# apache/incubator-predictionio

Measured on AMD Instinct MI355X. Metric: als_ratings_per_sec, higher is better.
Workload: dtype fp32; 1 GPU; model=als_rank64_implicit, global_batch=250000000, users=12500000, items=10000000, parallelism=dp1

## Files before the change

### predictionio_amd/ops/als.py

```python

from __future__ import annotations

from typing import Optional, Tuple

import torch

SUPPORTED_RANKS = (16, 32, 64, 128)


def pad_rank(f: int) -> int:
    for s in SUPPORTED_RANKS:
        if f <= s:
            return s
    raise ValueError(f"rank {f} > 128 not supported")


def gramian(Y: torch.Tensor) -> torch.Tensor:
    return Y.t() @ Y


def woodbury_lv(Y: torch.Tensor, YtY: torch.Tensor,
                lam: float) -> tuple:
    f = Y.shape[1]
    eye = torch.eye(f, dtype=Y.dtype, device=Y.device)
    B = YtY + lam * eye
    L = torch.linalg.cholesky(B)
    Linv = torch.linalg.solve_triangular(L, eye, upper=False)
    V = (Y @ Linv.mT).contiguous()
    import os as _os
    if (_os.environ.get("PIO_ALS_STAGE_BF16") == "1" and Y.is_cuda):
        V = V.to(torch.bfloat16).contiguous()
    return Linv, V


def als_solve(indptr: torch.Tensor, indices: torch.Tensor,
              values: torch.Tensor, Y: torch.Tensor,
              YtY: Optional[torch.Tensor] = None,
              lam: float = 0.01, alpha: float = 1.0,
              implicit: bool = False, wr_scale: bool = True,
              lv: Optional[tuple] = None,
              row_range: Optional[Tuple[int, int]] = None,
              out: Optional[torch.Tensor] = None) -> torch.Tensor:
    if implicit:
        wr_scale = False
        if YtY is None:
            YtY = gramian(Y)
    if row_range is not None:
        lo, hi = row_range
        indptr = indptr[lo:hi + 1]
    if Y.is_cuda:
        from predictionio_amd.ops import hip_ext
        ext = hip_ext()
        f = Y.shape[1]
        pf = pad_rank(f)
        Yp = (Y if pf == f
              else torch.nn.functional.pad(Y, (0, pf - f))).contiguous()
        YtYp = None
        if YtY is not None:
            YtYp = (YtY if pf == f
                    else torch.nn.functional.pad(YtY, (0, pf - f, 0, pf - f))
                    ).contiguous()
        ip, ix, vv = (indptr.contiguous(), indices.contiguous(),
                      values.contiguous())
        if ix.numel():
            mx = int(ix.max())
            if mx >= Y.shape[0] or int(ix.min()) < 0:
                raise ValueError(
                    f"CSR column id out of range: [{int(ix.min())}, {mx}]"
                    f" vs {Y.shape[0]} factor rows")
        direct_out = (out if out is not None and pf == f
                      and out.is_contiguous() else None)
        if implicit and pf <= 128:
            if lv is not None:
                Linv, V = lv
            else:
                Linv, V = woodbury_lv(Yp, YtYp, lam)
            import os as _os
            if _os.environ.get("PIO_ALS_STAGE_BF16") == "1" \
                    and V.dtype == torch.float32:
                V = V.to(torch.bfloat16).contiguous()
            Z = ext.als_solve(ip, ix, vv, Yp, YtYp, V, float(lam),
                              float(alpha), True, False, 1, None)
            if direct_out is not None:
                X = direct_out
                torch.matmul(Z, Linv, out=X)
            else:
                X = (Z @ Linv).contiguous()
            ext.als_solve(ip, ix, vv, Yp, YtYp, None, float(lam),
                          float(alpha), True, False, 2, X)
        else:
            X = ext.als_solve(ip, ix, vv, Yp, YtYp, None, float(lam),
                              float(alpha), bool(implicit), bool(wr_scale),
                              0, direct_out)
        res = X[:, :f].contiguous() if pf != f else X
        if out is not None and res.data_ptr() != out.data_ptr():
            out.copy_(res)
            return out
        return res
    res = als_solve_ref(indptr, indices, values, Y, YtY, lam, alpha,
                        implicit, wr_scale)
    if out is not None:
        out.copy_(res)
        return out
    return res


def prepare_lv(Y: torch.Tensor, YtY: torch.Tensor, lam: float):
    f = Y.shape[1]
    pf = pad_rank(f)
    Yp = (Y if pf == f
          else torch.nn.functional.pad(Y, (0, pf - f))).contiguous()
    YtYp = (YtY if pf == f
            else torch.nn.functional.pad(YtY, (0, pf - f, 0, pf - f))
            ).contiguous()
    return woodbury_lv(Yp, YtYp, lam)


def als_solve_ref(indptr, indices, values, Y, YtY=None, lam=0.01, alpha=1.0,
                  implicit=False, wr_scale=True) -> torch.Tensor:
    n_rows = indptr.shape[0] - 1
    f = Y.shape[1]
    X = torch.zeros((n_rows, f), dtype=Y.dtype, device=Y.device)
    eye = torch.eye(f, dtype=Y.dtype, device=Y.device)
    ip = indptr.tolist()
    for r in range(n_rows):
        s, e = ip[r], ip[r + 1]
        nnz = e - s
        if implicit:
            A = (YtY if YtY is not None else gramian(Y)).clone()
            b = torch.zeros(f, dtype=Y.dtype, device=Y.device)
            if nnz:
                cols = indices[s:e].long()
                Yr = Y[cols]
                v = values[s:e]
                A = A + (Yr.t() * (alpha * v)) @ Yr
                b = Yr.t() @ (1.0 + alpha * v)
            A = A + lam * eye
        else:
            if nnz == 0:
                continue
            cols = indices[s:e].long()
            Yr = Y[cols]
            v = values[s:e]
            A = Yr.t() @ Yr + lam * (nnz if wr_scale else 1.0) * eye
            b = Yr.t() @ v
        X[r] = torch.linalg.solve(A, b)
    return X


def build_csr(rows: torch.Tensor, cols: torch.Tensor, vals: torch.Tensor,
              n_rows: int) -> Tuple[torch.Tensor, torch.Tensor, torch.Tensor]:
    order = torch.argsort(rows)
    r = rows[order]
    indices = cols[order].to(torch.int32)
    values = vals[order].to(torch.float32)
    counts = torch.bincount(r.long(), minlength=n_rows)
    indptr = torch.zeros(n_rows + 1, dtype=torch.int64, device=rows.device)
    torch.cumsum(counts, 0, out=indptr[1:])
    return indptr, indices, values


def aggregate_ratings(rows: torch.Tensor, cols: torch.Tensor,
                      vals: torch.Tensor, n_cols: int,
                      mode: str = "sum"):
    key = rows.long() * n_cols + cols.long()
    if mode == "sum":
        uk, inv = torch.unique(key, return_inverse=True)
        out = torch.zeros(uk.numel(), dtype=torch.float32, device=vals.device)
        out.scatter_add_(0, inv, vals.float())
    elif mode == "latest":
        sk, order = torch.sort(key, stable=True)
        last = torch.ones(sk.numel(), dtype=torch.bool, device=key.device)
        last[:-1] = sk[1:] != sk[:-1]
        uk = sk[last]
        out = vals[order][last].float()
    else:
        raise ValueError(mode)
    return (uk // n_cols).to(rows.dtype), (uk % n_cols).to(cols.dtype), out
```

### predictionio_amd/ops/build.py

```python

from __future__ import annotations

import os
import subprocess
import sys
import sysconfig

OPS_DIR = os.path.dirname(os.path.abspath(__file__))
CSRC = os.path.join(OPS_DIR, "csrc")
SO_PATH = os.path.join(OPS_DIR, "_pio_hip.so")
SOURCES = ["bindings.cpp", "als_kernels.hip", "topk_kernels.hip",
           "topk_mfma.hip"]
HEADERS = ["topk_common.h"]
ARCH = os.environ.get("PYTORCH_ROCM_ARCH", "gfx950")


def _torch_paths():
    import torch
    root = os.path.dirname(torch.__file__)
    return {
        "includes": [
            os.path.join(root, "include"),
            os.path.join(root, "include", "torch", "csrc", "api", "include"),
        ],
        "libdir": os.path.join(root, "lib"),
        "abi": int(torch._C._GLIBCXX_USE_CXX11_ABI),
    }


def needs_build() -> bool:
    if not os.path.exists(SO_PATH):
        return True
    so_mtime = os.path.getmtime(SO_PATH)
    for s in SOURCES + HEADERS:
        if os.path.getmtime(os.path.join(CSRC, s)) > so_mtime:
            return True
    return False


def build(force: bool = False, verbose: bool = True) -> str:
    if not force and not needs_build():
        return SO_PATH
    tp = _torch_paths()
    py_include = sysconfig.get_paths()["include"]
    hipcc = os.environ.get("HIPCC", "hipcc")
    cmd = [
        hipcc, f"--offload-arch={ARCH}", "-O3", "-std=c++17", "-fPIC",
        "-shared",
        "-DTORCH_EXTENSION_NAME=_pio_hip",
        "-DTORCH_API_INCLUDE_EXTENSION_H",
        f"-D_GLIBCXX_USE_CXX11_ABI={tp['abi']}",
        "-D__HIP_PLATFORM_AMD__=1", "-DUSE_ROCM=1",
        "-Wno-deprecated-declarations", "-Wno-unused-result",
        f"-I{py_include}",
    ]
    for inc in tp["includes"]:
        cmd.append(f"-I{inc}")
    cmd += [os.path.join(CSRC, s) for s in SOURCES]
    cmd += [
        f"-L{tp['libdir']}", f"-Wl,-rpath,{tp['libdir']}",
        "-ltorch", "-ltorch_cpu", "-ltorch_python", "-ltorch_hip",
        "-lc10", "-lc10_hip", "-lamdhip64",
        "-o", SO_PATH,
    ]
    if verbose:
        print("[ops.build]", " ".join(cmd), file=sys.stderr)
    subprocess.run(cmd, check=True)
    return SO_PATH


if __name__ == "__main__":
    build(force="--force" in sys.argv)
```

### predictionio_amd/ops/csrc/als_kernels.hip

```cpp

#include <hip/hip_runtime.h>

#define CHUNK 16

__device__ __forceinline__ void wave_sync() {
  __builtin_amdgcn_wave_barrier();
}

typedef __attribute__((ext_vector_type(4))) float f32x4_t;
typedef __attribute__((ext_vector_type(2))) float f32x2_t;

__device__ __forceinline__ f32x2_t fma2(f32x2_t a, f32x2_t b, f32x2_t c) {
  return __builtin_elementwise_fma(a, b, c);
}

__device__ __forceinline__ int uniform_i32(int v) {
  return __builtin_amdgcn_readfirstlane(v);
}
__device__ __forceinline__ long long uniform_i64(long long v) {
  const unsigned int lo = (unsigned int)uniform_i32((int)(unsigned long long)v);
  const unsigned int hi =
      (unsigned int)uniform_i32((int)((unsigned long long)v >> 32));
  return (long long)(((unsigned long long)hi << 32) | lo);
}
__device__ __forceinline__ float lane_bcast(float v, int k) {
  return __int_as_float(__builtin_amdgcn_readlane(__float_as_int(v), k));
}


template <int F>
__global__ __launch_bounds__(256) void als_solve_kernel(
    const long long* __restrict__ indptr,
    const int* __restrict__ indices,
    const float* __restrict__ values,
    const float* __restrict__ Y,
    const float* __restrict__ YtY,
    float* __restrict__ X,
    int n_rows,
    float lambda,
    float alpha,
    int implicit_mode,
    int wr_scale,
    int skip_below)
{
  constexpr int TM = 4;
  constexpr int TILES = (F / TM) * (F / TM);
  constexpr int TPT = (TILES + 255) / 256;
  constexpr int NB = 16;
  static_assert(F % TM == 0, "F must be divisible by 4");
  static_assert(F % NB == 0, "F must be divisible by the panel width");

  __shared__ float ys[CHUNK][F + 1];
  __shared__ float ws_a[CHUNK];
  __shared__ float ws_b[CHUNK];
  __shared__ float As[F][F + 4];
  __shared__ float bs[F];
  __shared__ float dinv_all[F];

  const int tid = threadIdx.x;
  const int lane = tid & 63;
  const int wave = tid >> 6;

  for (long long row = blockIdx.x; row < n_rows; row += gridDim.x) {
    const long long start = indptr[row];
    const long long end = indptr[row + 1];
    const int nnz = (int)(end - start);
    if (nnz <= skip_below) continue;

    float acc[TPT][TM][TM];
#pragma unroll
    for (int t = 0; t < TPT; ++t)
#pragma unroll
      for (int i = 0; i < TM; ++i)
#pragma unroll
        for (int j = 0; j < TM; ++j) acc[t][i][j] = 0.f;

    for (int i = tid; i < F; i += 256) bs[i] = 0.f;

    for (int base = 0; base < nnz; base += CHUNK) {
      const int cn = min(CHUNK, nnz - base);
      __syncthreads();
      for (int e = tid; e < cn * F; e += 256) {
        const int c = e / F;
        const int k = e % F;
        const int col = indices[start + base + c];
        ys[c][k] = Y[(long long)col * F + k];
      }
      if (tid < cn) {
        const float r = values[start + base + tid];
        if (implicit_mode) {
          ws_a[tid] = alpha * r;
          ws_b[tid] = 1.f + alpha * r;
        } else {
          ws_a[tid] = 1.f;
          ws_b[tid] = r;
        }
      }
      __syncthreads();

      if (tid < F) {
        float bacc = 0.f;
        for (int c = 0; c < cn; ++c) bacc += ws_b[c] * ys[c][tid];
        bs[tid] += bacc;
      }

#pragma unroll
      for (int t = 0; t < TPT; ++t) {
        const int tile = tid + t * 256;
        if (TILES >= 256 || tile < TILES) {
          const int ti = (tile / (F / TM)) * TM;
          const int tj = (tile % (F / TM)) * TM;
          for (int c = 0; c < cn; ++c) {
            const float w = ws_a[c];
            float ya[TM], yb[TM];
#pragma unroll
            for (int i = 0; i < TM; ++i) ya[i] = ys[c][ti + i];
#pragma unroll
            for (int j = 0; j < TM; ++j) yb[j] = ys[c][tj + j];
#pragma unroll
            for (int i = 0; i < TM; ++i)
#pragma unroll
              for (int j = 0; j < TM; ++j)
                acc[t][i][j] = fmaf(w * ya[i], yb[j], acc[t][i][j]);
          }
        }
      }
    }
    __syncthreads();

#pragma unroll
    for (int t = 0; t < TPT; ++t) {
      const int tile = tid + t * 256;
      if (TILES >= 256 || tile < TILES) {
        const int ti = (tile / (F / TM)) * TM;
        const int tj = (tile % (F / TM)) * TM;
#pragma unroll
        for (int i = 0; i < TM; ++i)
#pragma unroll
          for (int j = 0; j < TM; ++j) {
            float v = acc[t][i][j];
            if (YtY != nullptr) v += YtY[(ti + i) * F + (tj + j)];
            As[ti + i][tj + j] = v;
          }
      }
    }
    __syncthreads();
    if (tid < F) {
      const float reg = wr_scale ? lambda * (float)nnz : lambda;
      As[tid][tid] += reg;
    }
    __syncthreads();

    for (int k0 = 0; k0 < F; k0 += NB) {
      if (wave == 0) {
        for (int kk = 0; kk < NB; ++kk) {
          const int kq = k0 + kk;
          wave_sync();
          float d = As[kq][kq];
          d = d > 0.f ? sqrtf(d) : 1e-20f;
          const float dinv = 1.f / d;
          if (lane == kk) {
            As[kq][kq] = d;
            dinv_all[kq] = dinv;
// ... 230 lines not shown
          for (int r = 0; r < 4; ++r)
            Lc[wave][ti * 16 + lg * 4 + r][tj * 16 + lq] =
                accm[ti][tj][r];
      wave_sync();
#pragma unroll
      for (int m = 0; m < F; ++m) ap[m >> 1][m & 1] = Lc[wave][m][lane];
      wave_sync();
    } else {
    float yn[PD], vn[PD];
#pragma unroll
    for (int p = 0; p < PD; ++p) {
      if (p < nnz) {
        const int col = indices[start + p];
        yn[p] = lane < F ? Y[(long long)col * F + lane] : 0.f;
        vn[p] = values[start + p];
      }
    }
    for (int c0 = 0; c0 < nnz; c0 += PD) {
#pragma unroll
      for (int p = 0; p < PD; ++p) {
        const int c = c0 + p;
        if (c >= nnz) break;
        const float ycur = yn[p];
        const float vcur = vn[p];
        if (lane < F) ys[wave][p][lane] = ycur;
        wave_sync();
        if (c + PD < nnz) {
          const int ncol = indices[start + c + PD];
          if (lane < F) yn[p] = Y[(long long)ncol * F + lane];
          vn[p] = values[start + c + PD];
        }
        float w_a, w_b;
        if (implicit_mode) {
          w_a = alpha * vcur;
          w_b = 1.f + alpha * vcur;
        } else {
          w_a = 1.f;
          w_b = vcur;
        }
        b_reg = fmaf(w_b, ycur, b_reg);
        const float wyj = w_a * ycur;
        const f32x2_t wyj2 = {wyj, wyj};
#pragma unroll
        for (int q = 0; q < F / 4; ++q) {
          const f32x4_t y4 =
              *reinterpret_cast<const f32x4_t*>(&ys[wave][p][4 * q]);
          ap[2 * q + 0] = fma2(wyj2, y4.lo, ap[2 * q + 0]);
          ap[2 * q + 1] = fma2(wyj2, y4.hi, ap[2 * q + 1]);
        }
        wave_sync();
      }
    }

    }

    if (YtY != nullptr && lane < F) {
#pragma unroll
      for (int q = 0; q < F / 4; ++q) {
        const f32x4_t t4 = *reinterpret_cast<const f32x4_t*>(
            &YtY[(long long)lane * F + 4 * q]);
        ap[2 * q + 0] += t4.lo;
        ap[2 * q + 1] += t4.hi;
      }
    }
    {
      const float reg = wr_scale ? lambda * (float)nnz : lambda;
#pragma unroll
      for (int m = 0; m < F; ++m)
        if (m == ln) ap[m >> 1][m & 1] += reg;
    }

    float dl = 0.f;
#pragma unroll
    for (int k = 0; k < F; ++k) {
      float lkk = lane_bcast(ap[k >> 1][k & 1], k);
      lkk = lkk > 1e-30f ? lkk : 1e-30f;
      const float dinv = rsqrtf(lkk);
      const float ljk = ln > k ? ap[k >> 1][k & 1] * dinv : 0.f;
      dl = ln == k ? dinv : dl;
      Lc[wave][k][lane < F ? lane : F] = ljk;
      ap[k >> 1][k & 1] = ljk;
      wave_sync();
      const f32x2_t nl2 = {-ljk, -ljk};
#pragma unroll
      for (int m4 = (k + 1) & ~3; m4 < F; m4 += 4) {
        const f32x4_t lq =
            *reinterpret_cast<const f32x4_t*>(&Lc[wave][k][m4]);
        const f32x2_t lh[2] = {lq.lo, lq.hi};
#pragma unroll
        for (int h = 0; h < 2; ++h) {
          const int m2 = m4 + 2 * h;
          if (m2 > k)
            ap[m2 >> 1] = fma2(nl2, lh[h], ap[m2 >> 1]);
          else if (m2 == k)
            ap[m2 >> 1][1] = fmaf(-ljk, lh[h][1], ap[m2 >> 1][1]);
        }
      }
      wave_sync();
    }

#pragma unroll
    for (int k = 0; k < F; ++k) {
      const float zk = lane_bcast(b_reg * dl, k);
      b_reg = fmaf(-ap[k >> 1][k & 1], zk, b_reg);
    }
    b_reg *= dl;
    {
      float4 lq = {0.f, 0.f, 0.f, 0.f};
#pragma unroll
      for (int k = F - 1; k >= 0; --k) {
        if ((k & 3) == 3 && lane < F)
          lq = *reinterpret_cast<const float4*>(&Lc[wave][lane][k & ~3]);
        const float xk = lane_bcast(b_reg * dl, k);
        const float lv = (k & 3) == 0 ? lq.x
                         : (k & 3) == 1 ? lq.y
                         : (k & 3) == 2 ? lq.z : lq.w;
        b_reg = fmaf(ln < k ? -lv : 0.f, xk, b_reg);
      }
      b_reg *= dl;
    }

    if (lane < F) X[row * (long long)F + lane] = b_reg;
  }
}


#define WOODBURY_MAX_NNZ 32


template <int F, int NW, int NLO, bool BF16S = false>
__global__ __launch_bounds__(128, NW > 24 ? 5 : 6) void als_woodbury_kernel(
    const long long* __restrict__ indptr,
    const int* __restrict__ indices,
    const float* __restrict__ values,
    const float* __restrict__ Y,
    const float* __restrict__ V,
    float* __restrict__ X,
    int n_rows,
    float lambda,
    float alpha,
    int implicit_mode,
    int wr_scale,
    unsigned long long* prof)
{
  constexpr int FP = F + 4;
  constexpr int FPH = F + 8;
  const int lane = threadIdx.x & 63;
  const int wave = uniform_i32((int)(threadIdx.x >> 6));

  __shared__ float Yl[2][NW][BF16S ? (FPH / 2) : FP];
  constexpr int MP = NW + 4;
  __shared__ float M[2][NW][MP];
  __shared__ float tv[2][NW];
  __shared__ float dv[2][NW];

  float* yl = &Yl[wave][0][0];
  unsigned short* ylh = reinterpret_cast<unsigned short*>(yl);
  const float* src = implicit_mode ? V : Y;
  const unsigned short* srch = reinterpret_cast<const unsigned short*>(V);

  for (long long row = (long long)blockIdx.x * 2 + wave; row < n_rows;
       row += (long long)gridDim.x * 2) {
    const long long start = uniform_i64(indptr[row]);
    const int n = uniform_i32((int)(indptr[row + 1] - start));
    if (n > NW || n <= NLO) continue;
    if (n == 0 && NLO < 0) {
      for (int e = lane; e < F; e += 64)
        X[row * (long long)F + e] = 0.f;
      continue;
    }
    const bool probe = prof != nullptr && (row & 1023) == 0 && lane == 0;
    unsigned long long pt0 = 0, pt1 = 0, pt2 = 0, pt3 = 0;
    if (probe) pt0 = wall_clock64();

    if (lane < n)
      tv[wave][lane] = __int_as_float(indices[start + lane]);
    wave_sync();
    for (int c = 0; c < n; ++c) {
      const long long col = __float_as_int(tv[wave][c]);
      if constexpr (BF16S) {
        const unsigned int* srow = reinterpret_cast<const unsigned int*>(
            srch + col * F);
        unsigned int* drow =
            reinterpret_cast<unsigned int*>(ylh + c * FPH);
        for (int e = lane; e < F / 2; e += 64) drow[e] = srow[e];
      } else {
        for (int e = lane; e < F; e += 64)
          yl[c * FP + e] = src[col * F + e];
      }
    }
    if (lane < n) {
      const float r = values[start + lane];
      if (implicit_mode) {
        const float ar = alpha * r;
        const float d = sqrtf(ar > 1e-12f ? ar : 1e-12f);
        dv[wave][lane] = d;
        tv[wave][lane] = (1.f + ar) / d;
      } else {
        tv[wave][lane] = r;
      }
    }
    wave_sync();
    if (probe) pt1 = wall_clock64();

    const float reg = wr_scale ? lambda * (float)n : lambda;
    const int npairs = n * (n + 1) / 2;
    {
      int p = lane, i = 0;
      while (p >= n - i && i < n) { p -= n - i; ++i; }
      int j = i + p;
      for (int pp = lane; pp < npairs; pp += 64) {
        float dot;
        if constexpr (BF16S) {
          const uint4* yi8 = reinterpret_cast<const uint4*>(&ylh[i * FPH]);
          const uint4* yj8 = reinterpret_cast<const uint4*>(&ylh[j * FPH]);
          f32x4_t acc4 = {0.f, 0.f, 0.f, 0.f};
#pragma unroll
          for (int q = 0; q < F / 8; ++q) {
            const uint4 a = yi8[q];
            const uint4 b = yj8[q];
            const unsigned int av[4] = {a.x, a.y, a.z, a.w};
            const unsigned int bv[4] = {b.x, b.y, b.z, b.w};
#pragma unroll
            for (int t = 0; t < 4; ++t) {
              acc4.x = fmaf(__uint_as_float(av[t] << 16),
                            __uint_as_float(bv[t] << 16), acc4.x);
              acc4.y = fmaf(__uint_as_float(av[t] & 0xffff0000u),
                            __uint_as_float(bv[t] & 0xffff0000u), acc4.y);
            }
          }
          dot = acc4.x + acc4.y;
        } else {
          const f32x4_t* yi = reinterpret_cast<const f32x4_t*>(&yl[i * FP]);
          const f32x4_t* yj = reinterpret_cast<const f32x4_t*>(&yl[j * FP]);
          f32x4_t acc4 = {0.f, 0.f, 0.f, 0.f};
#pragma unroll
          for (int q = 0; q < F / 4; ++q) acc4 += yi[q] * yj[q];
          dot = acc4.x + acc4.y + acc4.z + acc4.w;
        }
        if (implicit_mode) {
          dot *= dv[wave][i] * dv[wave][j];
          if (i == j) dot += 1.f;
        } else if (i == j) {
          dot += reg;
        }
        M[wave][i][j] = dot;
        M[wave][j][i] = dot;
        j += 64;
        while (j >= n && i < n) { ++i; j -= n - i; }
      }
    }
    wave_sync();

    if (probe) pt2 = wall_clock64();
    const int ln = lane | (int)(start >> 63);
    f32x2_t mp[NW / 2];
    const float* mrow = &M[wave][lane < NW ? lane : NW - 1][0];
    const int wcol = lane < NW ? lane : NW;
#pragma unroll
    for (int q = 0; q < NW / 4; ++q) {
      const f32x4_t r4 = *reinterpret_cast<const f32x4_t*>(&mrow[4 * q]);
      mp[2 * q + 0] = lane < n ? r4.lo : f32x2_t{0.f, 0.f};
      mp[2 * q + 1] = lane < n ? r4.hi : f32x2_t{0.f, 0.f};
    }
    float t = lane < n ? tv[wave][lane] : 0.f;
    float dl = 0.f;
    wave_sync();
#pragma unroll
    for (int k = 0; k < NW; ++k) {
      if (k < n) {
        float mkk = lane_bcast(mp[k >> 1][k & 1], k);
        mkk = mkk > 1e-30f ? mkk : 1e-30f;
        const float dinv = rsqrtf(mkk);
        const float ljk = ln > k ? mp[k >> 1][k & 1] * dinv : 0.f;
        dl = ln == k ? dinv : dl;
        mp[k >> 1][k & 1] = ljk;
        M[wave][k][wcol] = ljk;
        wave_sync();
        const f32x2_t nl2 = {-ljk, -ljk};
#pragma unroll
        for (int j4 = (k + 1) & ~3; j4 < NW; j4 += 4) {
          const f32x4_t q4 =
              *reinterpret_cast<const f32x4_t*>(&M[wave][k][j4]);
          const f32x2_t qh[2] = {q4.lo, q4.hi};
#pragma unroll
          for (int h = 0; h < 2; ++h) {
            const int j2 = j4 + 2 * h;
            if (j2 > k)
              mp[j2 >> 1] = fma2(nl2, qh[h], mp[j2 >> 1]);
            else if (j2 == k)
              mp[j2 >> 1][1] = fmaf(-ljk, qh[h][1], mp[j2 >> 1][1]);
          }
        }
        wave_sync();
      }
    }
#pragma unroll
    for (int k = 0; k < NW; ++k) {
      if (k < n) {
        const float zk = lane_bcast(t * dl, k);
        t = fmaf(-mp[k >> 1][k & 1], zk, t);
      }
    }
    t *= dl;
    wave_sync();
#pragma unroll
    for (int q = 0; q < NW / 4; ++q) {
      const f32x4_t r4 = *reinterpret_cast<const f32x4_t*>(&mrow[4 * q]);
      mp[2 * q + 0] = r4.lo;
      mp[2 * q + 1] = r4.hi;
    }
#pragma unroll
    for (int k = NW - 1; k >= 0; --k) {
      if (k < n) {
        const float xk = lane_bcast(t * dl, k);
        t = fmaf(ln < k ? -mp[k >> 1][k & 1] : 0.f, xk, t);
      }
    }
    t *= dl;
    if (implicit_mode) t *= dv[wave][lane < n ? lane : 0];
    if (lane < n) tv[wave][lane] = t;
    wave_sync();

    if (probe) pt3 = wall_clock64();
    for (int e = lane; e < F; e += 64) {
      float x = 0.f;
      for (int c = 0; c < n; ++c) {
        float ye;
        if constexpr (BF16S)
          ye = __uint_as_float((unsigned int)ylh[c * FPH + e] << 16);
        else
          ye = yl[c * FP + e];
        x = fmaf(tv[wave][c], ye, x);
      }
      X[row * (long long)F + e] = x;
    }
    if (probe) {
      const unsigned long long pt4 = wall_clock64();
      atomicAdd(&prof[0], pt1 - pt0);
      atomicAdd(&prof[1], pt2 - pt1);
      atomicAdd(&prof[2], pt3 - pt2);
      atomicAdd(&prof[3], pt4 - pt3);
      atomicAdd(&prof[4], 1ull);
    }
    wave_sync();
  }
}


template <int F, int NW, int NLO, bool BF16S = false>
__global__ __launch_bounds__(128, 3) void als_woodbury2_kernel(
    const long long* __restrict__ indptr,
    const int* __restrict__ indices,
    const float* __restrict__ values,
    const float* __restrict__ Y,
    const float* __restrict__ V,
    float* __restrict__ X,
    int n_rows,
    float lambda,
    float alpha,
// ... 370 lines not shown
```

### predictionio_amd/ops/csrc/bindings.cpp

```cpp

#include <torch/extension.h>

#include <ATen/hip/HIPContext.h>
#include <ATen/hip/impl/HIPGuardImplMasqueradingAsCUDA.h>
#include <ATen/hip/impl/HIPStreamMasqueradingAsCUDA.h>
#include <hip/hip_runtime.h>

extern "C" void launch_als_solve(
    const long long* indptr, const int* indices, const float* values,
    const float* Y, const float* YtY, const float* V, float* X,
    int n_rows, int f, float lambda, float alpha,
    int implicit_mode, int wr_scale, int which,
    unsigned long long* prof, hipStream_t stream);

extern "C" void launch_topk_score(
    const float* Xq, const float* Y, const uint8_t* item_mask,
    const long long* ban_indptr, const int* ban_indices,
    float* out_val, int* out_idx,
    int B, long long N, int f, int K, int n_slices, int item_base,
    unsigned long long* prof,
    const int* item_cats, const int* query_cats, int cw,
    hipStream_t stream);

extern "C" void launch_topk_mfma(
    const unsigned short* Xq, const unsigned short* Y,
    const uint8_t* item_mask, const long long* ban_indptr,
    const int* ban_indices, float* out_val, int* out_idx,
    int B, long long N, int f, int K, int n_slices, int item_base,
    unsigned long long* prof, unsigned* th_g,
    const int* item_cats, const int* query_cats, int cw,
    hipStream_t stream);

namespace {

void check_cuda_f32(const torch::Tensor& t, const char* name) {
  TORCH_CHECK(t.is_cuda(), name, " must be on GPU");
  TORCH_CHECK(t.is_contiguous(), name, " must be contiguous");
  TORCH_CHECK(t.scalar_type() == torch::kFloat32, name, " must be fp32");
}

bool supported_rank(int64_t f) {
  return f == 16 || f == 32 || f == 64 || f == 128;
}

int check_cats(const c10::optional<torch::Tensor>& item_cats,
               const c10::optional<torch::Tensor>& query_cats,
               int64_t B, int64_t N, bool has_prof) {
  TORCH_CHECK(item_cats.has_value() == query_cats.has_value(),
              "item_cats and query_cats must be given together");
  if (!item_cats.has_value()) return 0;
  TORCH_CHECK(!has_prof, "prof cannot be combined with category filters");
  TORCH_CHECK(item_cats->is_cuda() && item_cats->is_contiguous() &&
                  item_cats->scalar_type() == torch::kInt32 &&
                  item_cats->dim() == 2,
              "item_cats must be a contiguous [N, W] i32 GPU tensor");
  TORCH_CHECK(query_cats->is_cuda() && query_cats->is_contiguous() &&
                  query_cats->scalar_type() == torch::kInt32 &&
                  query_cats->dim() == 2,
              "query_cats must be a contiguous [B, W] i32 GPU tensor");
  const int64_t W = item_cats->size(1);
  TORCH_CHECK(W == 1 || W == 2 || W == 4,
              "category words W must be 1, 2 or 4, got ", W);
  TORCH_CHECK(item_cats->size(0) == N, "item_cats must have N rows");
  TORCH_CHECK(query_cats->size(0) == B && query_cats->size(1) == W,
              "query_cats must be [B, W] with item_cats' W");
  return (int)W;
}

struct TopkArgs {
  const uint8_t* mask = nullptr;
  const long long* ban_indptr = nullptr;
  const int* ban_indices = nullptr;
  unsigned long long* prof = nullptr;
  const int* item_cats = nullptr;
  const int* query_cats = nullptr;
  int cw = 0;
};

TopkArgs check_topk_args(const c10::optional<torch::Tensor>& item_mask,
                         const c10::optional<torch::Tensor>& ban_indptr,
                         const c10::optional<torch::Tensor>& ban_indices,
                         const c10::optional<torch::Tensor>& prof,
                         const c10::optional<torch::Tensor>& item_cats,
                         const c10::optional<torch::Tensor>& query_cats,
                         int64_t B, int64_t N) {
  TopkArgs a;
  a.cw = check_cats(item_cats, query_cats, B, N, prof.has_value());
  if (a.cw) {
    a.item_cats = item_cats->data_ptr<int>();
    a.query_cats = query_cats->data_ptr<int>();
  }
  if (item_mask.has_value()) {
    TORCH_CHECK(item_mask->is_cuda() && item_mask->is_contiguous() &&
                    item_mask->scalar_type() == torch::kUInt8,
                "item_mask must be contiguous u8 GPU");
    TORCH_CHECK(item_mask->size(0) == N, "item_mask size mismatch");
    a.mask = item_mask->data_ptr<uint8_t>();
  }
  if (ban_indptr.has_value()) {
    TORCH_CHECK(ban_indices.has_value(), "ban_indices required with ban_indptr");
    TORCH_CHECK(ban_indptr->is_cuda() && ban_indptr->is_contiguous() &&
                ban_indptr->scalar_type() == torch::kInt64);
    TORCH_CHECK(ban_indices->is_cuda() && ban_indices->is_contiguous() &&
                ban_indices->scalar_type() == torch::kInt32);
    TORCH_CHECK(ban_indptr->size(0) == B + 1, "ban_indptr must be B+1");
    a.ban_indptr = reinterpret_cast<const long long*>(
        ban_indptr->data_ptr<int64_t>());
    a.ban_indices = ban_indices->data_ptr<int>();
  }
  if (prof.has_value()) {
    TORCH_CHECK(prof->is_cuda() && prof->is_contiguous() &&
                    prof->scalar_type() == torch::kUInt64 &&
                    prof->numel() >= 5,
                "prof must be a contiguous u64[5] GPU tensor");
    a.prof = reinterpret_cast<unsigned long long*>(
        prof->data_ptr<uint64_t>());
  }
  return a;
}

torch::Tensor als_solve(torch::Tensor indptr, torch::Tensor indices,
                        torch::Tensor values, torch::Tensor Y,
                        c10::optional<torch::Tensor> YtY,
                        c10::optional<torch::Tensor> V,
                        double lambda, double alpha,
                        bool implicit_mode, bool wr_scale,
                        int64_t which, c10::optional<torch::Tensor> out,
                        c10::optional<torch::Tensor> prof) {
  TORCH_CHECK(indptr.is_cuda() && indptr.scalar_type() == torch::kInt64 &&
                  indptr.is_contiguous(), "indptr must be contiguous i64 GPU");
  TORCH_CHECK(indices.is_cuda() && indices.scalar_type() == torch::kInt32 &&
                  indices.is_contiguous(), "indices must be contiguous i32 GPU");
  check_cuda_f32(values, "values");
  check_cuda_f32(Y, "Y");
  const int64_t f = Y.size(1);
  TORCH_CHECK(supported_rank(f), "rank must be one of 16/32/64/128, got ", f);
  const int64_t n_rows = indptr.size(0) - 1;
  TORCH_CHECK(indices.size(0) == values.size(0), "indices/values mismatch");
  const float* yty_ptr = nullptr;
  if (YtY.has_value()) {
    check_cuda_f32(*YtY, "YtY");
    TORCH_CHECK(YtY->size(0) == f && YtY->size(1) == f, "YtY must be f x f");
    yty_ptr = YtY->data_ptr<float>();
  }
  const float* v_ptr = nullptr;
  if (V.has_value()) {
    TORCH_CHECK(V->is_cuda() && V->is_contiguous() &&
                    (V->scalar_type() == torch::kFloat32 ||
                     V->scalar_type() == torch::kBFloat16),
                "V must be contiguous fp32/bf16 GPU");
    TORCH_CHECK(V->sizes() == Y.sizes(), "V must match Y shape");
    const bool env_bf16 = [] {
      const char* e = getenv("PIO_ALS_STAGE_BF16");
      return e != nullptr && e[0] == '1';
    }();
    TORCH_CHECK((V->scalar_type() == torch::kBFloat16) == env_bf16,
                "V dtype must match PIO_ALS_STAGE_BF16");
    v_ptr = reinterpret_cast<const float*>(V->data_ptr());
  }
  unsigned long long* prof_ptr = nullptr;
  if (prof.has_value()) {
    TORCH_CHECK(prof->is_cuda() && prof->is_contiguous() &&
                prof->scalar_type() == torch::kUInt64 &&
                prof->numel() >= 5,
                "prof must be a contiguous u64 GPU tensor of >= 5");
    prof_ptr = reinterpret_cast<unsigned long long*>(
        prof->data_ptr());
  }
  torch::Tensor X;
  if (out.has_value()) {
    check_cuda_f32(*out, "out");
    TORCH_CHECK(out->size(0) == n_rows && out->size(1) == f,
                "out must be n_rows x f");
    X = *out;
  } else {
    X = torch::empty({n_rows, f}, Y.options());
  }
  c10::hip::HIPGuardMasqueradingAsCUDA guard(Y.device());
  hipStream_t stream = c10::hip::getCurrentHIPStreamMasqueradingAsCUDA().stream();
  launch_als_solve(reinterpret_cast<const long long*>(indptr.data_ptr<int64_t>()), indices.data_ptr<int>(),
                   values.data_ptr<float>(), Y.data_ptr<float>(), yty_ptr,
                   v_ptr, X.data_ptr<float>(), (int)n_rows, (int)f, (float)lambda,
                   (float)alpha, implicit_mode ? 1 : 0, wr_scale ? 1 : 0,
                   (int)which, prof_ptr, stream);
  C10_HIP_CHECK(hipGetLastError());
  return X;
}

std::tuple<torch::Tensor, torch::Tensor> topk_score(
    torch::Tensor Xq, torch::Tensor Y, int64_t K, int64_t n_slices,
    c10::optional<torch::Tensor> item_mask,
    c10::optional<torch::Tensor> ban_indptr,
    c10::optional<torch::Tensor> ban_indices, int64_t item_base,
    c10::optional<torch::Tensor> prof,
    c10::optional<torch::Tensor> item_cats,
    c10::optional<torch::Tensor> query_cats) {
  check_cuda_f32(Xq, "Xq");
  check_cuda_f32(Y, "Y");
  const int64_t f = Y.size(1);
  TORCH_CHECK(supported_rank(f), "rank must be one of 16/32/64/128, got ", f);
  TORCH_CHECK(Xq.size(1) == f, "Xq/Y rank mismatch");
  TORCH_CHECK(K >= 1 && K <= 64, "K must be in [1, 64]");
  const int64_t B = Xq.size(0);
  const int64_t N = Y.size(0);
  TORCH_CHECK(n_slices >= 1);
  const TopkArgs a = check_topk_args(item_mask, ban_indptr, ban_indices, prof,
                                     item_cats, query_cats, B, N);
  auto out_val = torch::empty({B, n_slices * 4 * K}, Xq.options());
  auto out_idx = torch::empty({B, n_slices * 4 * K},
                              Xq.options().dtype(torch::kInt32));
  c10::hip::HIPGuardMasqueradingAsCUDA guard(Y.device());
  hipStream_t stream = c10::hip::getCurrentHIPStreamMasqueradingAsCUDA().stream();
  launch_topk_score(Xq.data_ptr<float>(), Y.data_ptr<float>(), a.mask,
                    a.ban_indptr, a.ban_indices, out_val.data_ptr<float>(),
                    out_idx.data_ptr<int>(), (int)B, (long long)N, (int)f,
                    (int)K, (int)n_slices, (int)item_base, a.prof,
                    a.item_cats, a.query_cats, a.cw, stream);
  C10_HIP_CHECK(hipGetLastError());
  return {out_val, out_idx};
}

std::tuple<torch::Tensor, torch::Tensor> topk_score_mfma(
    torch::Tensor Xq, torch::Tensor Y, int64_t K, int64_t n_slices,
    c10::optional<torch::Tensor> item_mask,
    c10::optional<torch::Tensor> ban_indptr,
    c10::optional<torch::Tensor> ban_indices, int64_t item_base,
    c10::optional<torch::Tensor> prof,
    c10::optional<torch::Tensor> item_cats,
    c10::optional<torch::Tensor> query_cats) {
  TORCH_CHECK(Xq.is_cuda() && Xq.is_contiguous() &&
                  Xq.scalar_type() == torch::kBFloat16,
              "Xq must be contiguous bf16 GPU");
  TORCH_CHECK(Y.is_cuda() && Y.is_contiguous() &&
                  Y.scalar_type() == torch::kBFloat16,
              "Y must be contiguous bf16 GPU");
  const int64_t f = Y.size(1);
  TORCH_CHECK(f == 32 || f == 64 || f == 128,
              "mfma rank must be one of 32/64/128, got ", f);
  TORCH_CHECK(Xq.size(1) == f, "Xq/Y rank mismatch");
  TORCH_CHECK(K >= 1 && K <= 64, "K must be in [1, 64]");
  const int64_t B = Xq.size(0);
  const int64_t N = Y.size(0);
  TORCH_CHECK(n_slices >= 1);
  const TopkArgs a = check_topk_args(item_mask, ban_indptr, ban_indices, prof,
                                     item_cats, query_cats, B, N);
  auto out_val = torch::empty({B, n_slices * K},
                              Xq.options().dtype(torch::kFloat32));
  auto out_idx = torch::empty({B, n_slices * K},
                              Xq.options().dtype(torch::kInt32));
  c10::hip::HIPGuardMasqueradingAsCUDA guard(Y.device());
  hipStream_t stream =
      c10::hip::getCurrentHIPStreamMasqueradingAsCUDA().stream();
  torch::Tensor th_g;
  unsigned* th_g_ptr = nullptr;
  const char* e_gth = getenv("PIO_TOPK_GTH");
  const bool gth = !(e_gth != nullptr && e_gth[0] == '0');
  if (gth) {
    th_g = torch::zeros({B}, Xq.options().dtype(torch::kInt32));
    th_g_ptr = reinterpret_cast<unsigned*>(th_g.data_ptr<int>());
  }
  launch_topk_mfma(
      reinterpret_cast<const unsigned short*>(Xq.data_ptr()),
      reinterpret_cast<const unsigned short*>(Y.data_ptr()), a.mask,
      a.ban_indptr, a.ban_indices, out_val.data_ptr<float>(),
      out_idx.data_ptr<int>(), (int)B, (long long)N, (int)f, (int)K,
      (int)n_slices, (int)item_base, a.prof, th_g_ptr, a.item_cats,
      a.query_cats, a.cw, stream);
  C10_HIP_CHECK(hipGetLastError());
  return {out_val, out_idx};
}

}

PYBIND11_MODULE(TORCH_EXTENSION_NAME, m) {
  m.doc() = "MI355X (gfx950) HIP kernels for predictionio_amd";
  m.def("als_solve", &als_solve, "Fused ALS Gramian+Cholesky half-iteration",
        py::arg("indptr"), py::arg("indices"), py::arg("values"),
        py::arg("Y"), py::arg("YtY") = py::none(), py::arg("V") = py::none(),
        py::arg("lambda_") = 0.01,
        py::arg("alpha") = 1.0, py::arg("implicit_mode") = false,
        py::arg("wr_scale") = true, py::arg("which") = 0,
        py::arg("out") = py::none(), py::arg("prof") = py::none());
  m.def("topk_score", &topk_score, "Fused masked top-K scoring",
        py::arg("Xq"), py::arg("Y"), py::arg("K"), py::arg("n_slices") = 64,
        py::arg("item_mask") = py::none(), py::arg("ban_indptr") = py::none(),
        py::arg("ban_indices") = py::none(), py::arg("item_base") = 0,
        py::arg("prof") = py::none(), py::arg("item_cats") = py::none(),
        py::arg("query_cats") = py::none());
  m.def("topk_score_mfma", &topk_score_mfma,
        "Fused masked top-K scoring on MFMA (bf16 in, fp32 accumulate)",
        py::arg("Xq"), py::arg("Y"), py::arg("K"), py::arg("n_slices") = 64,
        py::arg("item_mask") = py::none(), py::arg("ban_indptr") = py::none(),
        py::arg("ban_indices") = py::none(), py::arg("item_base") = 0,
        py::arg("prof") = py::none(), py::arg("item_cats") = py::none(),
        py::arg("query_cats") = py::none());
}
```

Measured before the change: 1.768 billion ratings/s.

## Add fp32 MFMA row-transform kernel and MFMA Gramian in ALS solver

Adds a custom HIP kernel that computes in[N,f]·W[f,f] with fp32 32x32x2 MFMA instructions and a persistent grid with prefetch of the next tile. It replaces the torch matmuls Y@Linv^T and Z@Linv in the implicit Woodbury path. It also switches the per-row small Gramian in the solve kernel to an MFMA outer-product path for wide windows (NW>=24) on the non-bf16 path. Both changes aim to cut the cost of the skinny GEMMs and the scalar pair loop. The risks are numerical differences and that a bespoke GEMM may not beat hipBLASLt for tall-skinny shapes.

```diff
diff --git a/predictionio_amd/ops/als.py b/predictionio_amd/ops/als.py
--- a/predictionio_amd/ops/als.py
+++ b/predictionio_amd/ops/als.py
@@ -19,6 +19,12 @@
     return Y.t() @ Y
 
 
+def row_transform(A: torch.Tensor, W: torch.Tensor,
+                  out: Optional[torch.Tensor] = None) -> torch.Tensor:
+    from predictionio_amd.ops import hip_ext
+    return hip_ext().als_row_transform(A.contiguous(), W.contiguous(), out)
+
+
 def woodbury_lv(Y: torch.Tensor, YtY: torch.Tensor,
                 lam: float) -> tuple:
     f = Y.shape[1]
@@ -26,7 +32,10 @@
     B = YtY + lam * eye
     L = torch.linalg.cholesky(B)
     Linv = torch.linalg.solve_triangular(L, eye, upper=False)
-    V = (Y @ Linv.mT).contiguous()
+    if Y.is_cuda:
+        V = row_transform(Y, Linv.mT.contiguous())
+    else:
+        V = (Y @ Linv.mT).contiguous()
     import os as _os
     if (_os.environ.get("PIO_ALS_STAGE_BF16") == "1" and Y.is_cuda):
         V = V.to(torch.bfloat16).contiguous()
@@ -81,11 +90,7 @@
                 V = V.to(torch.bfloat16).contiguous()
             Z = ext.als_solve(ip, ix, vv, Yp, YtYp, V, float(lam),
                               float(alpha), True, False, 1, None)
-            if direct_out is not None:
-                X = direct_out
-                torch.matmul(Z, Linv, out=X)
-            else:
-                X = (Z @ Linv).contiguous()
+            X = row_transform(Z, Linv, out=direct_out)
             ext.als_solve(ip, ix, vv, Yp, YtYp, None, float(lam),
                           float(alpha), True, False, 2, X)
         else:
diff --git a/predictionio_amd/ops/build.py b/predictionio_amd/ops/build.py
--- a/predictionio_amd/ops/build.py
+++ b/predictionio_amd/ops/build.py
@@ -9,8 +9,8 @@
 OPS_DIR = os.path.dirname(os.path.abspath(__file__))
 CSRC = os.path.join(OPS_DIR, "csrc")
 SO_PATH = os.path.join(OPS_DIR, "_pio_hip.so")
-SOURCES = ["bindings.cpp", "als_kernels.hip", "topk_kernels.hip",
-           "topk_mfma.hip"]
+SOURCES = ["bindings.cpp", "als_kernels.hip", "als_xform.hip",
+           "topk_kernels.hip", "topk_mfma.hip"]
 HEADERS = ["topk_common.h"]
 ARCH = os.environ.get("PYTORCH_ROCM_ARCH", "gfx950")
 
diff --git a/predictionio_amd/ops/csrc/als_kernels.hip b/predictionio_amd/ops/csrc/als_kernels.hip
--- a/predictionio_amd/ops/csrc/als_kernels.hip
+++ b/predictionio_amd/ops/csrc/als_kernels.hip
@@ -9,6 +9,7 @@
 
 typedef __attribute__((ext_vector_type(4))) float f32x4_t;
 typedef __attribute__((ext_vector_type(2))) float f32x2_t;
+typedef __attribute__((ext_vector_type(16))) float f32x16_t;
 
 __device__ __forceinline__ f32x2_t fma2(f32x2_t a, f32x2_t b, f32x2_t c) {
   return __builtin_elementwise_fma(a, b, c);
@@ -545,7 +546,8 @@
   constexpr int MP = NW + 4;
   __shared__ float M[2][NW][MP];
   __shared__ float tv[2][NW];
-  __shared__ float dv[2][NW];
+  __shared__ __attribute__((aligned(16)))
+  float dv[2][NW];
 
   float* yl = &Yl[wave][0][0];
   unsigned short* ylh = reinterpret_cast<unsigned short*>(yl);
@@ -597,8 +599,44 @@
     if (probe) pt1 = wall_clock64();
 
     const float reg = wr_scale ? lambda * (float)n : lambda;
-    const int npairs = n * (n + 1) / 2;
-    {
+    constexpr bool MFMA_G = !BF16S && NW >= 24;
+    if constexpr (MFMA_G) {
+      const int gj = lane & 31, gh = lane >> 5;
+      const f32x4_t* vq = reinterpret_cast<const f32x4_t*>(
+          &yl[(gj < NW ? gj : NW - 1) * FP + 4 * gh]);
+      f32x16_t acc = {0.f, 0.f, 0.f, 0.f, 0.f, 0.f, 0.f, 0.f,
+                      0.f, 0.f, 0.f, 0.f, 0.f, 0.f, 0.f, 0.f};
+#pragma unroll
+      for (int q = 0; q < F / 8; ++q) {
+        const f32x4_t a = vq[2 * q];
+        acc = __builtin_amdgcn_mfma_f32_32x32x2f32(a.x, a.x, acc, 0, 0, 0);
+        acc = __builtin_amdgcn_mfma_f32_32x32x2f32(a.y, a.y, acc, 0, 0, 0);
+        acc = __builtin_amdgcn_mfma_f32_32x32x2f32(a.z, a.z, acc, 0, 0, 0);
+        acc = __builtin_amdgcn_mfma_f32_32x32x2f32(a.w, a.w, acc, 0, 0, 0);
+      }
+      static_assert(NW % 4 == 0 && NW <= 32, "one 32x32 tile, whole quads");
+      const float dj = dv[wave][gj < NW ? gj : NW - 1];
+      const float dg = implicit_mode ? 1.f : reg;
+      f32x4_t dadd;
+#pragma unroll
+      for (int t = 0; t < 4; ++t) dadd[t] = (gj & 3) == t ? dg : 0.f;
+#pragma unroll
+      for (int b = 0; b < (NW + 7) / 8; ++b) {
+        const int c0 = 8 * b + 4 * gh;
+        if (gj < NW && c0 < NW) {
+          const f32x4_t d4 = *reinterpret_cast<const f32x4_t*>(&dv[wave][c0]);
+          const bool diag = (gj >> 2) == 2 * b + gh;
+          f32x4_t m4;
+#pragma unroll
+          for (int t = 0; t < 4; ++t) {
+            const float sc = implicit_mode ? dj * d4[t] : 1.f;
+            m4[t] = acc[4 * b + t] * sc + (diag ? dadd[t] : 0.f);
+          }
+          *reinterpret_cast<f32x4_t*>(&M[wave][gj][c0]) = m4;
+        }
+      }
+    } else {
+      const int npairs = n * (n + 1) / 2;
       int p = lane, i = 0;
       while (p >= n - i && i < n) { p -= n - i; ++i; }
       int j = i + p;
diff --git a/predictionio_amd/ops/csrc/als_xform.hip b/predictionio_amd/ops/csrc/als_xform.hip
--- /dev/null
+++ b/predictionio_amd/ops/csrc/als_xform.hip
@@ -0,0 +1,129 @@
+
+#include <hip/hip_runtime.h>
+
+typedef __attribute__((ext_vector_type(4))) float f32x4_t;
+typedef __attribute__((ext_vector_type(16))) float f32x16_t;
+
+template <int F, int NCT>
+__global__ __launch_bounds__(256) void als_xform_kernel(
+    const float* __restrict__ in, const float* __restrict__ W,
+    float* __restrict__ out, long long n_rows)
+{
+  constexpr int NQ = F / 8;
+  constexpr int TC = F < 32 ? F : 32;
+  constexpr int CG = (F / TC) / NCT;
+  constexpr int TPW = 4 / CG;
+  static_assert(CG * NCT * TC == F && TPW * CG == 4, "tile split");
+
+  const int lane = threadIdx.x & 63;
+  const int wave = __builtin_amdgcn_readfirstlane((int)(threadIdx.x >> 6));
+  const int r = lane & 31, h = lane >> 5;
+  const int cbase = (wave % CG) * NCT * TC;
+
+  float w[NCT][NQ * 4];
+#pragma unroll
+  for (int ct = 0; ct < NCT; ++ct)
+#pragma unroll
+    for (int q = 0; q < NQ; ++q)
+#pragma unroll
+      for (int t = 0; t < 4; ++t) {
+        const int k = 8 * q + 4 * h + t;
+        const float v = W[k * F + cbase + ct * TC + (r < TC ? r : 0)];
+        w[ct][4 * q + t] = r < TC ? v : 0.f;
+      }
+
+  const long long n_tiles = (n_rows + 31) / 32;
+  const long long stride = (long long)gridDim.x * TPW;
+  long long tile = (long long)blockIdx.x * TPW + wave / CG;
+  if (tile >= n_tiles) return;
+
+  auto row_ptr = [&](long long tl) {
+    long long row = tl * 32 + r;
+    row = row < n_rows ? row : n_rows - 1;
+    return reinterpret_cast<const f32x4_t*>(in + row * F + 4 * h);
+  };
+
+  f32x4_t a[NQ];
+  {
+    const f32x4_t* p = row_ptr(tile);
+#pragma unroll
+    for (int q = 0; q < NQ; ++q) a[q] = p[2 * q];
+  }
+
+  for (; tile < n_tiles; tile += stride) {
+    f32x4_t an[NQ];
+    const long long next = tile + stride;
+    if (next < n_tiles) {
+      const f32x4_t* p = row_ptr(next);
+#pragma unroll
+      for (int q = 0; q < NQ; ++q) an[q] = p[2 * q];
+    } else {
+#pragma unroll
+      for (int q = 0; q < NQ; ++q) an[q] = a[q];
+    }
+
+    f32x16_t acc[NCT];
+#pragma unroll
+    for (int ct = 0; ct < NCT; ++ct)
+#pragma unroll
+      for (int e = 0; e < 16; ++e) acc[ct][e] = 0.f;
+#pragma unroll
+    for (int q = 0; q < NQ; ++q)
+#pragma unroll
+      for (int t = 0; t < 4; ++t)
+#pragma unroll
+        for (int ct = 0; ct < NCT; ++ct)
+          acc[ct] = __builtin_amdgcn_mfma_f32_32x32x2f32(
+              w[ct][4 * q + t], a[q][t], acc[ct], 0, 0, 0);
+
+    const long long row = tile * 32 + r;
+    if (row < n_rows) {
+      float* orow = out + row * F + cbase + 4 * h;
+#pragma unroll
+      for (int ct = 0; ct < NCT; ++ct)
+#pragma unroll
+        for (int b = 0; b < TC / 8; ++b) {
+          const f32x4_t o = {acc[ct][4 * b + 0], acc[ct][4 * b + 1],
+                             acc[ct][4 * b + 2], acc[ct][4 * b + 3]};
+          *reinterpret_cast<f32x4_t*>(orow + ct * TC + 8 * b) = o;
+        }
+    }
+#pragma unroll
+    for (int q = 0; q < NQ; ++q) a[q] = an[q];
+  }
+}
+
+template <int F, int NCT>
+static void launch_xform(const float* in, const float* W, float* out,
+                         long long n_rows, int n_cu, hipStream_t stream) {
+  constexpr int TC = F < 32 ? F : 32;
+  constexpr int TPW = 4 / ((F / TC) / NCT);
+  static int wg_per_cu = 0;
+  if (wg_per_cu == 0) {
+    int nb = 0;
+    if (hipOccupancyMaxActiveBlocksPerMultiprocessor(
+            &nb, als_xform_kernel<F, NCT>, 256, 0) != hipSuccess || nb < 1)
+      nb = 1;
+    wg_per_cu = nb;
+  }
+  const long long n_tiles = (n_rows + 31) / 32;
+  const long long want = (n_tiles + TPW - 1) / TPW;
+  const long long cap = (long long)n_cu * wg_per_cu;
+  const int grid = (int)(want < cap ? want : cap);
+  hipLaunchKernelGGL((als_xform_kernel<F, NCT>), dim3(grid), dim3(256), 0,
+                     stream, in, W, out, n_rows);
+}
+
+extern "C" void launch_als_row_transform(
+    const float* in, const float* W, float* out, long long n_rows, int f,
+    int n_cu, hipStream_t stream)
+{
+  if (n_rows <= 0) return;
+  switch (f) {
+    case 16: launch_xform<16, 1>(in, W, out, n_rows, n_cu, stream); break;
+    case 32: launch_xform<32, 1>(in, W, out, n_rows, n_cu, stream); break;
+    case 64: launch_xform<64, 2>(in, W, out, n_rows, n_cu, stream); break;
+    case 128: launch_xform<128, 1>(in, W, out, n_rows, n_cu, stream); break;
+    default: break;
+  }
+}
diff --git a/predictionio_amd/ops/csrc/bindings.cpp b/predictionio_amd/ops/csrc/bindings.cpp
--- a/predictionio_amd/ops/csrc/bindings.cpp
+++ b/predictionio_amd/ops/csrc/bindings.cpp
@@ -12,6 +12,10 @@
     int n_rows, int f, float lambda, float alpha,
     int implicit_mode, int wr_scale, int which,
     unsigned long long* prof, hipStream_t stream);
+
+extern "C" void launch_als_row_transform(
+    const float* in, const float* W, float* out, long long n_rows, int f,
+    int n_cu, hipStream_t stream);
 
 extern "C" void launch_topk_score(
     const float* Xq, const float* Y, const uint8_t* item_mask,
@@ -183,6 +187,40 @@
                    v_ptr, X.data_ptr<float>(), (int)n_rows, (int)f, (float)lambda,
                    (float)alpha, implicit_mode ? 1 : 0, wr_scale ? 1 : 0,
                    (int)which, prof_ptr, stream);
+  C10_HIP_CHECK(hipGetLastError());
+  return X;
+}
+
+torch::Tensor als_row_transform(torch::Tensor in, torch::Tensor W,
+                                c10::optional<torch::Tensor> out) {
+  check_cuda_f32(in, "in");
+  check_cuda_f32(W, "W");
+  TORCH_CHECK(in.dim() == 2 && W.dim() == 2, "in and W must be 2-D");
+  const int64_t n_rows = in.size(0);
+  const int64_t f = in.size(1);
+  TORCH_CHECK(supported_rank(f), "rank must be one of 16/32/64/128, got ", f);
+  TORCH_CHECK(W.size(0) == f && W.size(1) == f, "W must be f x f");
+  TORCH_CHECK(W.device() == in.device(), "W must be on in's device");
+  torch::Tensor X;
+  if (out.has_value()) {
+    check_cuda_f32(*out, "out");
+    TORCH_CHECK(out->dim() == 2 && out->size(0) == n_rows &&
+                    out->size(1) == f, "out must be n_rows x f");
+    TORCH_CHECK(out->device() == in.device(), "out must be on in's device");
+    X = *out;
+  } else {
+    X = torch::empty({n_rows, f}, in.options());
+  }
+  if (n_rows == 0) return X;
+  TORCH_CHECK(reinterpret_cast<uintptr_t>(in.data_ptr()) % 16 == 0 &&
+                  reinterpret_cast<uintptr_t>(X.data_ptr()) % 16 == 0,
+              "in/out must be 16-byte aligned");
+  c10::hip::HIPGuardMasqueradingAsCUDA guard(in.device());
+  hipStream_t stream = c10::hip::getCurrentHIPStreamMasqueradingAsCUDA().stream();
+  const int n_cu = at::cuda::getCurrentDeviceProperties()->multiProcessorCount;
+  launch_als_row_transform(in.data_ptr<float>(), W.data_ptr<float>(),
+                           X.data_ptr<float>(), (long long)n_rows, (int)f,
+                           n_cu, stream);
   C10_HIP_CHECK(hipGetLastError());
   return X;
 }
@@ -281,6 +319,9 @@
         py::arg("alpha") = 1.0, py::arg("implicit_mode") = false,
         py::arg("wr_scale") = true, py::arg("which") = 0,
         py::arg("out") = py::none(), py::arg("prof") = py::none());
+  m.def("als_row_transform", &als_row_transform,
+        "out[N, f] = in[N, f] . W[f, f], fp32 MFMA row transform",
+        py::arg("in_"), py::arg("W"), py::arg("out") = py::none());
   m.def("topk_score", &topk_score, "Fused masked top-K scoring",
         py::arg("Xq"), py::arg("Y"), py::arg("K"), py::arg("n_slices") = 64,
         py::arg("item_mask") = py::none(), py::arg("ban_indptr") = py::none(),
```

After: 1.923 billion ratings/s, median of 6. 8.8% higher.
